# hitbc/panSVR

Measured on AMD Instinct MI355X. Metric: signal reads realigned/sec (150 bp PE); bit-exact CIGAR vs CPU ref, higher is better.
Workload: dtype u8/int32 (2-bit k-mers, 8-bit DP deltas, 32-bit scores); 1 GPU; configs[1]: 1000000 synthetic 150 bp PE signal read pairs per GPU vs 10000-anchor SV reference (11.8 Mbp), `panSVR aln` hot path; pairs_per_gpu=1000000, engines_per_gpu=1, in_process_rebases=0, index_hbm_bytes=2713674320, index_distribution=every rank uploads its own copy from host memory

## Files before the change

pansvr_amd/csrc/ksw_kernels.hip:

```cpp
#include <hip/hip_runtime.h>
#include <stdint.h>
#include "ksw_device.h"

namespace psvr {

__device__ __forceinline__ void write_ez(psvr_extz_t *o, const EzAcc &a, int n_cigar)
{
	o->max = a.max, o->zdropped = a.zdropped;
	o->max_q = a.max_q, o->max_t = a.max_t;
	o->mqe = a.mqe, o->mqe_t = a.mqe_t;
	o->mte = a.mte, o->mte_q = a.mte_q;
	o->score = a.score, o->n_cigar = n_cigar, o->reach_end = a.reach_end, o->reserved = 0;
}

__device__ __forceinline__ void wave_slot_take(int t, int tlen, const uint8_t *target, int neg_qe, int neg_qe2,
                                               int &u, int &v, int &x, int &y, int &x2, int &y2, int &s, int &H, int &tb)
{
	u = v = x = y = neg_qe, x2 = y2 = neg_qe2, s = 0, H = PSVR_KSW_NEG_INF;
	tb = t < tlen ? target[t] : 0;
}
template <int K, bool RING>
__device__ __forceinline__ void dp_wave_loop(const DpParams &P, const uint8_t *target, int lane, int qlen, int tlen, int w, int rowb, int n_rows,
                                             const uint8_t *QR, uint8_t *Pm, EzAcc &ez)
{
// ... 106 lines not shown
		last_st = st;
	}
}

template <int K>
__device__ __forceinline__ void dp_lean_loop(const DpParams &P, const uint8_t *target, int lane, int qlen, int tlen, int rowb, int n_rows,
                                             const uint8_t *QR, uint8_t *Pm, EzAcc &ez_out)
{
	const int neg_qe = s8(-P.q - P.e), neg_qe2 = s8(-P.q2 - P.e2);
	const int qe8 = s8(P.q + P.e), qe28 = s8(P.q2 + P.e2);
	const int with_cigar = !(P.flag & PSVR_EZ_SCORE_ONLY);
	int u[K], v[K], x[K], y[K], x2[K], y2[K], H[K], tb[K], mis[K];
#pragma unroll
	for (int c = 0; c < K; ++c) {
		const int t = c * 64 + lane;
		v[c] = x[c] = y[c] = neg_qe;
		x2[c] = y2[c] = neg_qe2;
		u[c] = dp_edge_gap(P, t);
		H[c] = -P.qe_pre;
		const int tc = t < tlen ? target[t] : 0;
		tb[c] = tc == P.m1 ? 0x100 : tc;
		mis[c] = tc == P.m1 ? P.sc_N : P.sc_mis;
	}
	__builtin_amdgcn_wave_barrier();
	int e_max = 0, e_max_t = -1, e_max_q = -1, e_mqe = PSVR_KSW_NEG_INF, e_mqe_t = -1, e_mte = PSVR_KSW_NEG_INF, e_mte_q = -1;
	int e_score = PSVR_KSW_NEG_INF, e_zd = 0, last_H = PSVR_KSW_NEG_INF;
	for (int r = 0; r < n_rows; ++r) {
		const int st0 = max(0, r - qlen + 1), en0 = min(tlen - 1, r);
		const int ur = dp_edge_gap(P, r);
		const int c_first = st0 >> 6, c_last = en0 >> 6;
		const int qbase = qlen - 1 - r;
		const unsigned prow = (unsigned)(r * rowb - (st0 & ~15));
		int h_prev = 0;
#pragma unroll
		for (int c = 0; c < K; ++c) {
			if (en0 > 0 && ((en0 - 1) >> 6) == c) h_prev = __builtin_amdgcn_readlane(H[c], (en0 - 1) & 63);
		}
		const int sel_t = en0 > 0 ? en0 : -1;
		int bh = (int)0x80000000;
		unsigned long long amask[K];
#pragma unroll
		for (int c = K - 1; c >= 0; --c) {
			amask[c] = 0;
			if (c < c_first || c > c_last) continue;
			const int t = c * 64 + lane;
			int cx = neg_qe, cv = ur, cx2 = neg_qe2;
			if (c > 0) {
				cx = __builtin_amdgcn_readlane(x[c - 1], 63);
				cv = __builtin_amdgcn_readlane(v[c - 1], 63);
				cx2 = __builtin_amdgcn_readlane(x2[c - 1], 63);
			}
			const int xt1 = dpp_wave_shr1(x[c], cx), vt1 = dpp_wave_shr1(v[c], cv), x2t1 = dpp_wave_shr1(x2[c], cx2);
			const int qb = QR[(unsigned)(qbase + t)];
			int sc = tb[c] == qb ? P.sc_mch : mis[c];
			sc = qb == P.m1 ? P.sc_N : sc;
			const int ut = u[c];
			int a = xt1 + vt1, b = y[c] + ut, a2 = x2t1 + vt1, b2 = y2[c] + ut;
			int z = max(max(sc, a), b);
			z = max(max(z, a2), b2);
			int d = 4;
			d = a2 == z ? 3 : d;
			d = b == z ? 2 : d;
			d = a == z ? 1 : d;
			d = sc == z ? 0 : d;
			z = min(z, P.sc_mch);
			const int un = z - vt1, vn = z - ut;
			const int zq = z - P.q, zq2 = z - P.q2;
			a -= zq, b -= zq, a2 -= zq2, b2 -= zq2;
			d |= (a > 0 ? 0x08 : 0) | (b > 0 ? 0x10 : 0) | (a2 > 0 ? 0x20 : 0) | (b2 > 0 ? 0x40 : 0);
			const int hn = t == sel_t ? h_prev + un : H[c] + vn;
			const bool act = (t >= st0) & (t <= en0);
			amask[c] = __ballot(act);
			if (act) {
				u[c] = un, v[c] = vn;
				x[c] = max(a, 0) - qe8, y[c] = max(b, 0) - qe8;
				x2[c] = max(a2, 0) - qe28, y2[c] = max(b2, 0) - qe28;
				H[c] = hn;
				if (with_cigar) Pm[prow + (unsigned)t] = (uint8_t)d;
				bh = max(bh, hn);
			}
		}
		const int max_H = wave_max_i32(bh);
		int n_top = 0, max_t = 0;
		unsigned long long top[K];
#pragma unroll
		for (int c = 0; c < K; ++c) {
			top[c] = 0;
			if (c < c_first || c > c_last) continue;
			top[c] = __ballot(H[c] == max_H) & amask[c];
			n_top += __popcll(top[c]);
			if (top[c]) max_t = c * 64 + __ffsll((unsigned long long)top[c]) - 1;
		}
		if (n_top != 1) {
			const int en1 = dp_diag_en1(st0, en0);
			unsigned bk = 0xffffffffu;
#pragma unroll
			for (int c = 0; c < K; ++c)
				if ((top[c] >> lane) & 1) bk = min(bk, dp_diag_rank<12>(c * 64 + lane, st0, en0, en1));
			max_t = dp_rank_col<12>(wave_min_u32(bk), st0, en0);
		}
		if (en0 == tlen - 1) {
			int H_en0 = 0;
#pragma unroll
			for (int c = 0; c < K; ++c)
				if ((en0 >> 6) == c) H_en0 = __builtin_amdgcn_readlane(H[c], en0 & 63);
			if (H_en0 > e_mte) e_mte = H_en0, e_mte_q = r - (((en0 + 16) & ~15) - 1);
			if (r == n_rows - 1) last_H = H_en0;
		}
		if (r - st0 == qlen - 1) {
			int H_st0 = 0;
#pragma unroll
			for (int c = 0; c < K; ++c)
				if ((st0 >> 6) == c) H_st0 = __builtin_amdgcn_readlane(H[c], st0 & 63);
			if (H_st0 > e_mqe) e_mqe = H_st0, e_mqe_t = st0;
		}
		if (max_H > e_max) {
			e_max = max_H, e_max_t = max_t, e_max_q = r - max_t;
		} else if (max_t >= e_max_t && r - max_t >= e_max_q) {
			const int tl = max_t - e_max_t, ql = (r - max_t) - e_max_q;
			const int l = tl > ql ? tl - ql : ql - tl;
			if (P.zdrop >= 0 && e_max - max_H > P.zdrop + l * P.e2) { e_zd = 1; break; }
		}
		if (r == n_rows - 1) e_score = last_H;
	}
	ez_out.max = e_max, ez_out.max_t = e_max_t, ez_out.max_q = e_max_q;
	ez_out.mqe = e_mqe, ez_out.mqe_t = e_mqe_t, ez_out.mte = e_mte, ez_out.mte_q = e_mte_q;
	ez_out.score = e_score, ez_out.zdropped = e_zd;
}

template <int K, bool PG, bool RING, int NW = kDpWaves>
__device__ __forceinline__ void extd2_wave_body(const DpBatch &B, const DpParams &P)
{
	extern __shared__ __align__(16) uint8_t lds_all[];
	const int wave = uni(threadIdx.x >> 6);
	const long long slot = (long long)blockIdx.x * NW + wave;
	if (slot >= B.n) return;
	uint8_t *lds = lds_all + (size_t)wave * B.lds_per_wave;
	const int pid = uni(B.idx[slot]);
	const int lane = threadIdx.x & 63;
	const int qlen = uni(B.qlen[pid]), tlen = uni(B.tlen[pid]);
	psvr_extz_t *out = B.ez + pid;
	EzAcc ez;
	ez.reset();
	if (P.skip || qlen <= 0 || tlen <= 0) {
		if (lane == 0) write_ez(out, ez, 0);
		return;
	}
	const uint8_t *query = B.qseq + uni64(B.q_off[pid]), *target = B.tseq + uni64(B.t_off[pid]);
	const int w = dp_band_w(qlen, tlen, P.w);
	const int rowb = uni(dp_n_col(qlen, tlen, P.w) * 16);
	const int n_rows = qlen + tlen - 1;
	const int qimg = (qlen + 16 + 15) & ~15;
	uint8_t *QR = lds;
	uint8_t *Pm = PG ? B.pslab + (uni64(B.p_off[pid]) << B.p_unit_shift) : lds + qimg;
	const int p_end = n_rows * rowb + 16;
	for (int i = lane; i < qimg; i += 64) QR[i] = i < qlen ? query[qlen - 1 - i] : 0;
	if (RING) {
		uint8_t *TG = lds + qimg;
		for (int i = lane; i < tlen; i += 64) TG[i] = target[i];
		dp_wave_loop<K, true>(P, TG, lane, qlen, tlen, w, rowb, n_rows, QR, Pm, ez);
	}
	else if (P.nowrap_ok && dp_band_never_binds(qlen, tlen, w)) dp_lean_loop<K>(P, target, lane, qlen, tlen, rowb, n_rows, QR, Pm, ez);
	else dp_wave_loop<K, false>(P, target, lane, qlen, tlen, w, rowb, n_rows, QR, Pm, ez);
	const int with_cigar = !(P.flag & PSVR_EZ_SCORE_ONLY);
	int n_cigar = 0;
	if (with_cigar) {
		if (PG) __threadfence_block();
		__builtin_amdgcn_wave_barrier();
		int i0, j0;
		if (trace_start(ez, P, qlen, tlen, i0, j0)) {
			uint32_t *stage_end = (uint32_t*)(Pm + p_end);
			n_cigar = traceback(i0, j0, qlen, tlen, w,
				[&](int r, int k) { return PG ? (int)__builtin_nontemporal_load(Pm + (size_t)r * rowb + k) : (int)Pm[r * rowb + k]; },
				[&](int k, uint32_t word) { if (lane == 0) stage_end[-1 - k] = word; });
			if (PG) __threadfence_block();
			__builtin_amdgcn_wave_barrier();
			uint32_t *dst = B.cigar + uni64(out->cigar_off);
			const bool rev = (P.flag & PSVR_EZ_REV_CIGAR) != 0;
			for (int m = lane; m < n_cigar; m += 64) {
				const uint32_t *src = rev ? stage_end - 1 - m : stage_end - n_cigar + m;
				dst[m] = PG ? __builtin_nontemporal_load(src) : *src;
			}
		}
	}
	if (lane == 0) write_ez(out, ez, n_cigar);
}
template <int K, bool PG>
__global__ __launch_bounds__(64 * kDpWaves) void extd2_reg_kernel(DpBatch B, DpParams P) { extd2_wave_body<K, PG, false>(B, P); }
template <int K>
__global__ __launch_bounds__(64 * kDpWaves) void extd2_ring_kernel(DpBatch B, DpParams P) { extd2_wave_body<K, true, true>(B, P); }
template __global__ void extd2_ring_kernel<3>(DpBatch, DpParams);
template __global__ void extd2_ring_kernel<4>(DpBatch, DpParams);
template <int K>
__global__ __launch_bounds__(64) void extd2_ring1_kernel(DpBatch B, DpParams P) { extd2_wave_body<K, true, true, 1>(B, P); }
template __global__ void extd2_ring1_kernel<3>(DpBatch, DpParams);
template __global__ void extd2_ring1_kernel<4>(DpBatch, DpParams);

template __global__ void extd2_reg_kernel<1, false>(DpBatch, DpParams);
template __global__ void extd2_reg_kernel<2, false>(DpBatch, DpParams);
template __global__ void extd2_reg_kernel<1, true>(DpBatch, DpParams);
template __global__ void extd2_reg_kernel<2, true>(DpBatch, DpParams);
template __global__ void extd2_reg_kernel<3, true>(DpBatch, DpParams);
template __global__ void extd2_reg_kernel<4, true>(DpBatch, DpParams);
template __global__ void extd2_reg_kernel<5, true>(DpBatch, DpParams);


__global__ __launch_bounds__(64) void extd2_tiny_kernel(DpBatch B, DpParams P, int max_rows)
{
	extern __shared__ __align__(16) uint32_t tiny_lds[];
	const int lane = threadIdx.x;
	const long long slot = (long long)blockIdx.x * 64 + lane;
	if (slot >= B.n) return;
	uint32_t *W0 = tiny_lds + lane, *W1 = tiny_lds + 16 * 64 + lane;
	uint8_t *PD = (uint8_t *)(tiny_lds + 2 * 16 * 64) + lane;
	const int pid = B.idx[slot];
	const int qlen = B.qlen[pid], tlen = B.tlen[pid];
	psvr_extz_t *out = B.ez + pid;
	EzAcc ez;
	ez.reset();
	if (P.skip || qlen <= 0 || tlen <= 0 || qlen > PSVR_DP_TINY_MAX || tlen > PSVR_DP_TINY_MAX || qlen + tlen - 1 > max_rows) { write_ez(out, ez, 0); return; }
	const uint8_t *query = B.qseq + B.q_off[pid], *target = B.tseq + B.t_off[pid];
	unsigned long long qp = 0, tp = 0;
	for (int i = 0; i < qlen; ++i) qp |= (unsigned long long)(query[i] & 15) << (4 * i);
	for (int i = 0; i < tlen; ++i) tp |= (unsigned long long)(target[i] & 15) << (4 * i);
	const int neg_qe = s8(-P.q - P.e), neg_qe2 = s8(-P.q2 - P.e2);
	const int qe8 = s8(P.q + P.e), qe28 = s8(P.q2 + P.e2);
	const int with_cigar = !(P.flag & PSVR_EZ_SCORE_ONLY);
	auto pack0 = [](int u, int v, int x, int y) { return (uint32_t)(u & 0xff) | (uint32_t)(v & 0xff) << 8 | (uint32_t)(x & 0xff) << 16 | (uint32_t)(y & 0xff) << 24; };
	auto pack1 = [](int x2, int y2, int h) { return (uint32_t)(x2 & 0xff) | (uint32_t)(y2 & 0xff) << 8 | (uint32_t)(h & 0xffff) << 16; };
	for (int t = 0; t < tlen; ++t) {
		W0[t * 64] = pack0(dp_edge_gap(P, t), neg_qe, neg_qe, neg_qe);
		W1[t * 64] = pack1(neg_qe2, neg_qe2, -P.qe_pre);
	}
	const int n_rows = qlen + tlen - 1;
	for (int r = 0; r < n_rows; ++r) {
		const int st0 = max(0, r - qlen + 1), en0 = min(tlen - 1, r);
		const int en1 = dp_diag_en1(st0, en0);
		int x1 = neg_qe, v1 = dp_edge_gap(P, r), x21 = neg_qe2, h1 = 0;
		if (st0 > 0) {
			const uint32_t a = W0[(st0 - 1) * 64], b = W1[(st0 - 1) * 64];
			v1 = s8(a >> 8), x1 = s8(a >> 16), x21 = s8(b), h1 = (int)(int16_t)(b >> 16);
		}
		int bh = (int)0x80000000, H_en0 = 0, H_st0 = 0;
		unsigned bk = 0xffffffffu;
		for (int t = st0; t <= en0; ++t) {
			const uint32_t a = W0[t * 64], b = W1[t * 64];
			const int ut = s8(a), vo = s8(a >> 8), xo = s8(a >> 16), yo = s8(a >> 24), x2o = s8(b), y2o = s8(b >> 8), ho = (int)(int16_t)(b >> 16);
			const int xt1 = x1, vt1 = v1, x2t1 = x21, hl = h1;
			x1 = xo, v1 = vo, x21 = x2o, h1 = ho;
			const int tc = (int)(tp >> (4 * t)) & 15, qc = (int)(qp >> (4 * (r - t))) & 15;
			int sc = tc == qc ? P.sc_mch : P.sc_mis;
			sc = (tc == P.m1 || qc == P.m1) ? P.sc_N : sc;
			int za = xt1 + vt1, zb = yo + ut, za2 = x2t1 + vt1, zb2 = y2o + ut;
			int z = max(max(sc, za), zb);
			z = max(max(z, za2), zb2);
			int d = 4;
			d = za2 == z ? 3 : d;
			d = zb == z ? 2 : d;
			d = za == z ? 1 : d;
			d = sc == z ? 0 : d;
			z = min(z, P.sc_mch);
			const int un = z - vt1, vn = z - ut;
			const int zq = z - P.q, zq2 = z - P.q2;
			za -= zq, zb -= zq, za2 -= zq2, zb2 -= zq2;
			d |= (za > 0 ? 0x08 : 0) | (zb > 0 ? 0x10 : 0) | (za2 > 0 ? 0x20 : 0) | (zb2 > 0 ? 0x40 : 0);
			const int hn = (t == en0 && en0 > 0) ? hl + un : ho + vn;
			W0[t * 64] = pack0(un, vn, max(za, 0) - qe8, max(zb, 0) - qe8);
			W1[t * 64] = pack1(max(za2, 0) - qe28, max(zb2, 0) - qe28, hn);
			if (with_cigar) PD[(r * 16 + t) * 64] = (uint8_t)d;
			if (t == en0) H_en0 = hn;
			if (t == st0) H_st0 = hn;
			const unsigned rank = dp_diag_rank<12>(t, st0, en0, en1);
			if (hn > bh || (hn == bh && rank < bk)) bh = hn, bk = rank;
		}
		const int max_t = dp_rank_col<12>(bk, st0, en0);
		if (ez.end_diagonal(r, qlen, tlen, st0, en0, H_st0, H_en0, bh, max_t, P.zdrop, P.e2)) break;
	}
	int n_cigar = 0;
	if (with_cigar) {
		int i0, j0;
		if (trace_start(ez, P, qlen, tlen, i0, j0)) {
			const int w = dp_band_w(qlen, tlen, P.w);
			n_cigar = traceback(i0, j0, qlen, tlen, w,
				[&](int r, int k) { return (int)PD[(r * 16 + k) * 64]; },
				[&](int k, uint32_t word) { (k < 16 ? W0[k * 64] : W1[(k - 16) * 64]) = word; });
			uint32_t *dst = B.cigar + out->cigar_off;
			const bool rev = (P.flag & PSVR_EZ_REV_CIGAR) != 0;
			for (int m = 0; m < n_cigar; ++m) {
				const int k = rev ? m : n_cigar - 1 - m;
				dst[m] = k < 16 ? W0[k * 64] : W1[(k - 16) * 64];
			}
		}
	}
	write_ez(out, ez, n_cigar);
}

static constexpr int kTeamWaves = 3;
template <int LANES, int CPL, int LEAN>
__global__ __launch_bounds__(64) __attribute__((amdgpu_waves_per_eu(kTeamWaves, 8))) void extd2_team_kernel(DpBatch B, DpParams P, TeamPlan T)
{
	static_assert(CPL == 4 || CPL == 8 || CPL == 16, "columns per lane: direction bytes go out as dwords");
	constexpr int SW = CPL * LANES, PB = 64 / LANES;
	constexpr int kNone = (int)0x80000000;
	const int lane = threadIdx.x, team = lane / LANES, ql = lane % LANES;
	__shared__ int sc_lut[64];
	{
		const int tcode = lane >> 3, qcode = lane & 7;
		sc_lut[lane] = 8 * ((tcode == P.m1 || qcode == P.m1) ? P.sc_N : (tcode == qcode ? P.sc_mch : P.sc_mis)) + 4;
	}
	__builtin_amdgcn_wave_barrier();
	int cls = 0;
	while (cls + 1 < T.n_classes && (int)blockIdx.x >= T.first_block[cls + 1]) ++cls;
	const int n_strips16 = T.n_strips16[cls];
	const long long slot = (long long)((int)blockIdx.x - T.first_block[cls]) * PB + team;
	const bool live = slot < T.count[cls];
	int pid = 0, qlen = 0, tlen = 0;
	if (live) pid = B.idx[T.first_slot[cls] + slot], qlen = B.qlen[pid], tlen = B.tlen[pid];
	const int n_strips = (n_strips16 * 16 + SW - 1) / SW;
	const int qmax = wave_max_i32(qlen > 0 ? qlen : 0);
	const int ksteps = uni(qmax + LANES - 1);
	const int k_last = uni(-wave_max_i32(live && qlen > 0 ? -qlen : (int)0x80000000)) - 1;
	const int R = ksteps, NR = qmax + SW * n_strips + 1;
	const unsigned long long need = dp_team_ws_bytes(qmax, n_strips16, LANES, CPL);
	const unsigned long long base = T.ws_base[cls] + (unsigned long long)((int)blockIdx.x - T.first_block[cls]) * T.ws_need[cls];
	const bool bad_shape = qlen <= 0 || tlen <= 0 || (tlen + SW - 1) / SW > n_strips;
	if (!live) return;
	if (base + need > B.ws_cap && B.err) *B.err = 20;
	if (P.skip || bad_shape || base + need > B.ws_cap) return;
	uint8_t *w0 = B.ws + base;
	const size_t offE = (size_t)(64 * CPL) * n_strips * R;
	uint8_t *const uE0 = w0 + offE, *const uE1 = w0 + offE + (size_t)4 * PB * NR;
	uint8_t *const uD = w0 + offE + (size_t)8 * PB * NR, *const uD23 = uD + (size_t)4 * PB * NR;
	const unsigned lc = (unsigned)CPL * (unsigned)lane, t4 = 4u * (unsigned)team;
	auto at4 = [=](uint8_t *ub, int r) -> int & { return *(int *)(ub + (size_t)r * (4 * PB) + t4); };
	auto atD2 = [=](int r) -> short & { return *(short *)(uD23 + (size_t)r * (4 * PB) + t4); };
	auto atD3 = [=](int r) -> short & { return *(short *)(uD23 + (size_t)r * (4 * PB) + t4 + 2); };
	const uint8_t *query = B.qseq + B.q_off[pid], *target = B.tseq + B.t_off[pid];
	const int with_cigar = !(P.flag & PSVR_EZ_SCORE_ONLY);
	const int neg_qe = s8(-P.q - P.e), neg_qe2 = s8(-P.q2 - P.e2);
	const int x_init = 8 * neg_qe + 3, y_init = 8 * neg_qe + 2, x2_init = 8 * neg_qe2 + 1, y2_init = 8 * neg_qe2;
	const int z_cap = 8 * P.sc_mch + 7;
	const int q_m8 = 8 * P.q - 8, q2_m8 = 8 * P.q2 - 8;
	const int cx = 8 - 8 * s8(P.q + P.e), cx2 = 8 - 8 * s8(P.q2 + P.e2);
	const int long_thres = P.long_thres, ur_short = s8(-P.e), ur_at = s8(P.long_diff), ur_long = s8(-P.e2);
	auto ur_of = [=](int r) { return r == 0 ? neg_qe : r < long_thres ? ur_short : r == long_thres ? ur_at : ur_long; };
	auto h_above = [&](int t) {
		int h = -P.qe_pre;
		const int lt = P.long_thres;
		if (t >= 1) {
			if (lt >= 1) h += t < lt ? t * s8(-P.e) : (lt - 1) * s8(-P.e) + s8(P.long_diff) + (t - lt) * s8(-P.e2);
			else h += t * s8(-P.e2);
		}
		return h;
	};
	auto frank = [](int p) { return (((p << 12) + p) & 0x3fff) ^ 0x3fff; };
	const int ns = (tlen + SW - 1) / SW;
	for (int sv = 0; sv < ns; ++sv) {
		const int s = uni(sv);
		const int c0 = SW * s;
		const int ncols = tlen - c0 < SW ? tlen - c0 : SW;
		const int jb = CPL * ql, cb = c0 + jb;
		const int jx = tlen - 1 - cb;
		const bool own = (unsigned)jx < (unsigned)CPL;
		int U[CPL], V[CPL], X[CPL], Y[CPL], X2[CPL], Y2[CPL], H[CPL], TC[CPL];
		int M[CPL], K[CPL], G[CPL];
		bool inr[CPL];
#pragma unroll
		for (int jj = 0; jj < CPL; ++jj) {
			U[jj] = 8 * ur_of(cb + jj);
			V[jj] = 8 * neg_qe, X[jj] = x_init, Y[jj] = y_init, X2[jj] = x2_init, Y2[jj] = y2_init;
			H[jj] = 8 * h_above(cb + jj);
			inr[jj] = jb + jj < ncols;
			TC[jj] = inr[jj] ? (target[cb + jj] & 7) * 32 : 0;
			M[jj] = kNone, G[jj] = frank(cb + jj);
			const int d = cb + jj - ql;
			const int st = max(0, d - qlen + 1), en = min(tlen - 1, d);
			K[jj] = st + ((en - st) & ~3) - cb;
		}
		(void)M, (void)K, (void)G;
		uint8_t *const Ein = (s & 1) ? uE0 : uE1, *const Eout = (s & 1) ? uE1 : uE0;
		unsigned e_prev = 0;
		unsigned dirw[CPL / 4];
		int d_cur = kNone, out_prev = kNone;
		if (s > 0) {
			e_prev = (unsigned)at4(Ein, 0);
			if (!LEAN && 0 <= ksteps - LANES) d_cur = at4(uD, c0);
		}
		unsigned q_cur = ql == 0 ? query[0] : 0u;
		for (int kv = 0; kv < LANES - 1; ++kv) {
			const int k = uni(kv);
#define TEAM_MASKED 1
#define TEAM_TOPROW 1
#include "ksw_row_step.inc"
#undef TEAM_MASKED
#undef TEAM_TOPROW
		}
		{
			const int k = LANES - 1;
#define TEAM_MASKED 0
#define TEAM_TOPROW 1
#include "ksw_row_step.inc"
#undef TEAM_MASKED
#undef TEAM_TOPROW
		}
		for (int kv = LANES; kv < ksteps; ++kv) {
			const int k = uni(kv);
#define TEAM_MASKED 0
#define TEAM_TOPROW 0
#include "ksw_row_step.inc"
#undef TEAM_MASKED
#undef TEAM_TOPROW
		}
		if (with_cigar) {
			uint32_t *const dst = (uint32_t *)(w0 + (size_t)(s * R + ksteps - 1) * (64 * CPL) + lc);
#pragma unroll
			for (int g = 0; g < CPL / 4; ++g) dst[g] = dirw[g];
		}
		if (LEAN) { __threadfence_block(); continue; }
		if (LANES > 1) {
			const int inc = __builtin_amdgcn_update_dpp(kNone, out_prev, 0x101, 0xf, 0xf, false);
			const int m0 = __builtin_amdgcn_update_dpp(kNone, M[0], 0x101, 0xf, 0xf, false);
			M[CPL - 2] = max(M[CPL - 2], ql == LANES - 1 ? kNone : inc);
			M[CPL - 1] = max(M[CPL - 1], ql == LANES - 1 ? kNone : m0);
		}
#pragma unroll
		for (int jj = 0; jj < CPL; ++jj)
			if (jj > 0 || ql == 0) at4(uD, ksteps - ql + cb + jj) = M[jj];
		__threadfence_block();
	}
}

static constexpr int kFinishWaves = 8;
template <int LANES, int CPL, int LEAN>
__global__ __launch_bounds__(64) __attribute__((amdgpu_waves_per_eu(1, kFinishWaves))) void extd2_team_finish_kernel(DpBatch B, DpParams P, TeamPlan T)
{
	constexpr int SW = CPL * LANES, PB = 64 / LANES, kWinRows = 8;
	__shared__ uint32_t win[kWinRows * (CPL / 4) * 64];
	const int lane = threadIdx.x, team = lane % PB;
	const int tb = (int)((blockIdx.x * 64u + (unsigned)lane) / (unsigned)PB);
	const bool in_grid = tb < T.first_block[T.n_classes];
	int cls = 0;
	while (cls + 1 < T.n_classes && tb >= T.first_block[cls + 1]) ++cls;
	const int n_strips16 = T.n_strips16[cls];
	const long long slot = (long long)(tb - T.first_block[cls]) * PB + team;
	const bool live = in_grid && slot < T.count[cls];
	int pid = 0, qlen = 0, tlen = 0;
	if (live) pid = B.idx[T.first_slot[cls] + slot], qlen = B.qlen[pid], tlen = B.tlen[pid];
	const int n_strips = (n_strips16 * 16 + SW - 1) / SW;
	int qmax = qlen > 0 ? qlen : 0;
#pragma unroll
	for (int d = 1; d < PB; d <<= 1) qmax = max(qmax, __shfl_xor(qmax, d, 64));
	const int ksteps = qmax + LANES - 1;
	const int R = ksteps, NR = qmax + SW * n_strips + 1;
	const unsigned long long need = dp_team_ws_bytes(qmax, n_strips16, LANES, CPL);
	const unsigned long long base = T.ws_base[cls] + (unsigned long long)(tb - T.first_block[cls]) * T.ws_need[cls];
	if (!live) return;
	psvr_extz_t *out = B.ez + pid;
	EzAcc ez;
	ez.reset();
	const bool bad_shape = qlen <= 0 || tlen <= 0 || (tlen + SW - 1) / SW > n_strips;
	if (P.skip || bad_shape || base + need > B.ws_cap) { write_ez(out, ez, 0); return; }
	uint8_t *w0 = B.ws + base;
	const size_t offE = (size_t)(64 * CPL) * n_strips * R;
	uint8_t *const uD = w0 + offE + (size_t)8 * PB * NR, *const uD23 = uD + (size_t)4 * PB * NR;
	const unsigned t4 = 4u * (unsigned)team;
	auto at4 = [=](uint8_t *ub, int r) -> int & { return *(int *)(ub + (size_t)r * (4 * PB) + t4); };
	const int with_cigar = !(P.flag & PSVR_EZ_SCORE_ONLY);
	const int n_rows = qlen + tlen - 1;
	bool stop = false;
	for (int r0 = 0; r0 < n_rows && !stop; r0 += 8) {
		int kd[8], h2[8], h3[8];
#pragma unroll
		for (int u = 0; u < 8; ++u) {
			const int r = min(r0 + u, n_rows - 1);
			const int w23 = at4(uD23, r);
			kd[u] = LEAN ? 0 : at4(uD, r), h2[u] = (int)(short)(w23 & 0xffff), h3[u] = w23 >> 16;
		}
#pragma unroll
		for (int u = 0; u < 8; ++u) {
			const int r = r0 + u;
			if (r >= n_rows || stop) continue;
			const int st0 = max(0, r - qlen + 1), en0 = min(tlen - 1, r);
			const int key = kd[u];
			const int max_H = key >> 16;
			const int H_en0 = h2[u];
			const int max_t = H_en0 == max_H ? en0 : st0 + ((0x7fff - (key & 0xffff)) & 4095);
			if (en0 == tlen - 1 && H_en0 > ez.mte) ez.mte = H_en0, ez.mte_q = r - (((en0 + 16) & ~15) - 1);
			if (r - st0 == qlen - 1 && h3[u] > ez.mqe) ez.mqe = h3[u], ez.mqe_t = st0;
			if (!LEAN && ez.apply_zdrop(max_H, r, max_t, P.zdrop, P.e2)) stop = true;
			else if (r == n_rows - 1) ez.score = H_en0;
		}
	}
	int n_cigar = 0;
	if (with_cigar) {
		int i0, j0;
		if (trace_start(ez, P, qlen, tlen, i0, j0)) {
			const int w = dp_band_w(qlen, tlen, P.w);
			const uint8_t *pb = w0 + team * SW;
			uint32_t *stage = (uint32_t *)(w0 + offE) + team;
			int win_row = -1, win_grp = -1;
			n_cigar = traceback(i0, j0, qlen, tlen, w,
				[&](int r, int k) {
					const int t = k + (max(0, r - qlen + 1) & ~15), row = r - t, grp = t / CPL;
					if (grp != win_grp || row > win_row || row <= win_row - kWinRows) {
						const int s = grp / LANES, gl = grp % LANES;
						const uint8_t *src = pb + (size_t)(s * R + row + gl) * (64 * CPL) + gl * CPL;
						uint32_t tmp[kWinRows][CPL / 4];
#pragma unroll
						for (int d = 0; d < kWinRows; ++d)
#pragma unroll
							for (int u = 0; u < CPL / 4; ++u) tmp[d][u] = d <= row ? ((const uint32_t *)(src - (size_t)d * (64 * CPL)))[u] : 0u;
#pragma unroll
						for (int d = 0; d < kWinRows; ++d)
#pragma unroll
							for (int u = 0; u < CPL / 4; ++u) win[(d * (CPL / 4) + u) * 64 + lane] = tmp[d][u];
						win_row = row, win_grp = grp;
					}
					const int x = t % CPL;
					const unsigned b = (win[((win_row - row) * (CPL / 4) + (x >> 2)) * 64 + lane] >> (8 * (x & 3))) & 0xffu, n = ~b;
					return (int)((4u - ((b >> 4) & 7u)) | ((n >> 3) & 1u) << 3 | ((n >> 2) & 1u) << 4 | ((n >> 1) & 1u) << 5 | (n & 1u) << 6);
				},
				[&](int k, uint32_t word) { stage[(size_t)k * PB] = word; });
			uint32_t *dst = B.cigar + out->cigar_off;
			const bool rev = (P.flag & PSVR_EZ_REV_CIGAR) != 0;
			for (int m = 0; m < n_cigar; ++m) dst[m] = stage[(size_t)(rev ? m : n_cigar - 1 - m) * PB];
		}
	}
	write_ez(out, ez, n_cigar);
}
template __global__ void extd2_team_kernel<kDpTeamLanes, kDpTeamCpl, 0>(DpBatch, DpParams, TeamPlan);
template __global__ void extd2_team_finish_kernel<kDpTeamLanes, kDpTeamCpl, 0>(DpBatch, DpParams, TeamPlan);
template __global__ void extd2_team_kernel<kDpTeamLanes, kDpTeamCpl, 1>(DpBatch, DpParams, TeamPlan);
template __global__ void extd2_team_finish_kernel<kDpTeamLanes, kDpTeamCpl, 1>(DpBatch, DpParams, TeamPlan);

struct GenK {
	int neg_qe, neg_qe2, qe8, qe28;
	int qe;
	uint8_t qe2b, max_scb, qb8;
	int with_cigar, approx_max, right;
};
__device__ __forceinline__ GenK gen_consts(const DpParams &P)
{
	GenK k;
	k.neg_qe = s8(-P.q - P.e), k.neg_qe2 = s8(-P.q2 - P.e2), k.qe8 = s8(P.q + P.e), k.qe28 = s8(P.q2 + P.e2);
	k.qe = P.q + P.e;
	k.qe2b = (uint8_t)((P.q + P.e) * 2), k.max_scb = (uint8_t)(P.mat[0] + (P.q + P.e) * 2), k.qb8 = (uint8_t)P.q;
	k.with_cigar = !(P.flag & PSVR_EZ_SCORE_ONLY), k.approx_max = !!(P.flag & PSVR_EZ_APPROX_MAX);
	k.right = k.with_cigar && (P.flag & PSVR_EZ_RIGHT);
	return k;
}

template <int VAR, class IDX>
struct GenImage {
	static constexpr int NARR = VAR == 0 ? 7 : 5;
	uint8_t *base;
	IDX T, img;
	int8_t *u8, *v8, *x8, *y8, *x28, *y28, *sa;
	uint8_t *sf, *qr;
	int32_t *H;
	__device__ __forceinline__ void place(uint8_t *at, int qlen, int tlen)
	{
		base = at;
		T = ((IDX)tlen + 15) / 16 * 16;
		const IDX QL = ((IDX)qlen + 15) / 16 * 16;
		u8 = (int8_t*)at, v8 = u8 + T, x8 = v8 + T, y8 = x8 + T;
		x28 = VAR == 0 ? y8 + T : nullptr, y28 = VAR == 0 ? x28 + T : nullptr;
		sa = VAR == 0 ? y28 + T : y8 + T;
		sf = (uint8_t*)(sa + T), qr = sf + T;
		img = NARR * T + T + QL + 16;
		H = (int32_t*)(at + ((img + 15) & ~(IDX)15));
	}
	__device__ __forceinline__ void init(int tid, int nthreads, const uint8_t *query, const uint8_t *target, int qlen, int tlen, const GenK &k) const
	{
		for (IDX i = tid; i < img; i += nthreads) {
			const IDX a = i / T;
			uint8_t val = 0;
			if (VAR == 0) { if (a < 4) val = (uint8_t)k.neg_qe; else if (a < 6) val = (uint8_t)k.neg_qe2; }
			if (a == NARR) { const IDX t = i - NARR * T; val = t < tlen ? target[t] : 0; }
			if (a > NARR)  { const IDX j = i - (NARR + 1) * T; val = j < qlen ? query[qlen - 1 - j] : 0; }
			base[i] = val;
		}
		for (IDX i = tid; i < T; i += nthreads) H[i] = PSVR_KSW_NEG_INF;
	}
	__device__ __forceinline__ int du(const GenK &k, int t) const { return VAR == 0 ? (int)u8[t] : (int)(uint8_t)u8[t] - k.qe; }
	__device__ __forceinline__ int dv(const GenK &k, int t) const { return VAR == 0 ? (int)v8[t] : (int)(uint8_t)v8[t] - k.qe; }
	__device__ __forceinline__ int h_first(const GenK &k, const DpParams &P) const { return dv(k, 0) - (VAR == 0 ? P.qe_pre : k.qe); }
};

template <int VAR, class IMG>
__device__ __forceinline__ void gen_left_boundary(const IMG &I, const GenK &k, const DpParams &P, int r, int st, int last_st, int last_en, int &x1, int &x21, int &v1)
{
	x21 = 0;
	if (VAR == 0) {
		if (st > 0) {
			if (st - 1 >= last_st && st - 1 <= last_en) x1 = I.x8[st - 1], x21 = I.x28[st - 1], v1 = I.v8[st - 1];
			else x1 = k.neg_qe, x21 = k.neg_qe2, v1 = k.neg_qe;
		} else x1 = k.neg_qe, x21 = k.neg_qe2, v1 = dp_edge_gap(P, r);
	} else {
		if (st > 0) {
			if (st - 1 >= last_st && st - 1 <= last_en) x1 = I.x8[st - 1], v1 = I.v8[st - 1];
			else x1 = v1 = 0;
		} else x1 = 0, v1 = r ? s8(P.q) : 0;
	}
}

template <int VAR, class IMG>
__device__ __forceinline__ void gen_row_override(const IMG &I, const GenK &k, const DpParams &P, int r)
{
	if (VAR == 0) I.y8[r] = k.neg_qe, I.y28[r] = k.neg_qe2, I.u8[r] = dp_edge_gap(P, r);
	else I.y8[r] = 0, I.u8[r] = r ? (int8_t)k.qb8 : 0;
}

struct GenLate { int t, sc; };
template <bool DEFER, class IMG>
__device__ __forceinline__ GenLate gen_scores(const IMG &I, const DpParams &P, int qlen, int r, int st0, int en0, int tid, int nthreads)
{
	const uint8_t *qrr = I.qr + (qlen - 1 - r);
	GenLate late = {-1, 0};
	if (!(P.flag & PSVR_EZ_GENERIC_SC)) {
		const int fresh_end = dp_fresh_end(st0, en0);
		for (int t = st0 + tid; t <= fresh_end; t += nthreads) {
			const uint8_t sq = I.sf[t], sq2 = qrr[t];
			int sc = sq == sq2 ? P.sc_mch : P.sc_mis;
			if (sq == (uint8_t)P.m1 || sq2 == (uint8_t)P.m1) sc = P.sc_N;
			if (!DEFER || t < I.T) I.sa[t] = (int8_t)sc;
			else late.t = t, late.sc = sc;
		}
	} else {
		for (int t = st0 + tid; t <= en0; t += nthreads) I.sa[t] = P.mat[I.sf[t] * P.m + qrr[t]];
	}
	return late;
}

struct GenCell { int u, v, x, y, x2, y2, d; };
template <int VAR, class IMG>
__device__ __forceinline__ GenCell gen_cell(const IMG &I, const GenK &k, const DpParams &P, int t, int st, int x1, int x21, int v1)
{
	GenCell c = {0, 0, 0, 0, 0, 0, 0};
	int d = 0;
	if (VAR == 0) {
		int xt1 = t == st ? x1 : (int)I.x8[t - 1], vt1 = t == st ? v1 : (int)I.v8[t - 1], x2t1 = t == st ? x21 : (int)I.x28[t - 1];
		int z = I.sa[t], ut = I.u8[t];
		int a = s8(xt1 + vt1), b = s8(I.y8[t] + ut), a2 = s8(x2t1 + vt1), b2 = s8(I.y28[t] + ut);
		if (!k.right) {
			if (a > z)  d = 1, z = a;
			if (b > z)  d = 2, z = b;
			if (a2 > z) d = 3, z = a2;
			if (b2 > z) d = 4, z = b2;
		} else {
			d = z > a ? 0 : 1;  z = z > a ? z : a;
			d = z > b ? d : 2;  z = z > b ? z : b;
			d = z > a2 ? d : 3; z = z > a2 ? z : a2;
			d = z > b2 ? d : 4; z = z > b2 ? z : b2;
		}
		z = min(z, P.sc_mch);
		c.u = z - vt1, c.v = z - ut;
		int tmp = s8(z - P.q);
		a = s8(a - tmp), b = s8(b - tmp);
		tmp = s8(z - P.q2);
		a2 = s8(a2 - tmp), b2 = s8(b2 - tmp);
		c.x = max(a, 0) - k.qe8, c.y = max(b, 0) - k.qe8, c.x2 = max(a2, 0) - k.qe28, c.y2 = max(b2, 0) - k.qe28;
		if (!k.right) d |= (a > 0 ? 0x08 : 0) | (b > 0 ? 0x10 : 0) | (a2 > 0 ? 0x20 : 0) | (b2 > 0 ? 0x40 : 0);
		else d |= (a >= 0 ? 0x08 : 0) | (b >= 0 ? 0x10 : 0) | (a2 >= 0 ? 0x20 : 0) | (b2 >= 0 ? 0x40 : 0);
	} else {
		const int j = t - st;
		unsigned x1w = (unsigned)x1, v1w = (unsigned)v1;
		uint8_t xt1 = j == 0 ? 0 : (uint8_t)I.x8[t - 1], vt1 = j == 0 ? 0 : (uint8_t)I.v8[t - 1];
		if (j < 4) xt1 |= (uint8_t)(x1w >> (8 * j)), vt1 |= (uint8_t)(v1w >> (8 * j));
		uint8_t z = (uint8_t)((uint8_t)I.sa[t] + k.qe2b), a = (uint8_t)(xt1 + vt1), ut = (uint8_t)I.u8[t], b = (uint8_t)((uint8_t)I.y8[t] + ut);
		if (!k.with_cigar) {
			z = (int8_t)z > 0 ? z : 0; z = z > a ? z : a;
		} else if (!k.right) {
			d = (int8_t)a > (int8_t)z ? 1 : 0;
			z = (int8_t)z > 0 ? z : 0; z = z > a ? z : a;
			if ((int8_t)b > (int8_t)z) d = 2;
		} else {
			d = (int8_t)z > (int8_t)a ? 0 : 1;
			z = (int8_t)z > 0 ? z : 0; z = z > a ? z : a;
			if (!((int8_t)z > (int8_t)b)) d = 2;
		}
		z = z > b ? z : b;
		z = z < k.max_scb ? z : k.max_scb;
		c.u = (uint8_t)(z - vt1), c.v = (uint8_t)(z - ut);
		z = (uint8_t)(z - k.qb8);
		a = (uint8_t)(a - z), b = (uint8_t)(b - z);
		if (!k.right) {
			c.x = (int8_t)a > 0 ? (int8_t)a : 0; d |= (int8_t)a > 0 ? 0x08 : 0;
			c.y = (int8_t)b > 0 ? (int8_t)b : 0; d |= (int8_t)b > 0 ? 0x10 : 0;
		} else {
			c.x = (int8_t)a < 0 ? 0 : (int8_t)a; d |= (int8_t)a < 0 ? 0 : 0x08;
			c.y = (int8_t)b < 0 ? 0 : (int8_t)b; d |= (int8_t)b < 0 ? 0 : 0x10;
		}
	}
	c.d = d;
	return c;
}
template <int VAR, class IMG>
__device__ __forceinline__ void gen_store_cell(const IMG &I, int t, const GenCell &c)
{
	I.u8[t] = (int8_t)c.u, I.v8[t] = (int8_t)c.v, I.x8[t] = (int8_t)c.x, I.y8[t] = (int8_t)c.y;
	if (VAR == 0) I.x28[t] = (int8_t)c.x2, I.y28[t] = (int8_t)c.y2;
}

template <class IMG>
__device__ __forceinline__ int gen_h_en0(const IMG &I, const GenK &k, int en0)
{
	const int uen = I.du(k, en0), ven = I.dv(k, en0);
	return en0 > 0 ? I.H[en0 - 1] + uen : I.H[en0] + ven;
}
template <int RS, class IMG>
__device__ __forceinline__ void gen_exact_h_partial(const IMG &I, const GenK &k, int st0, int en0, int h_en0, int tid, int nthreads, int &bh, unsigned &bk)
{
	const int en1 = dp_diag_en1(st0, en0);
	bh = (int)0x80000000, bk = 0xffffffffu;
	for (int t = st0 + tid; t <= en0; t += nthreads) {
		const int h = t == en0 ? h_en0 : I.H[t] + I.dv(k, t);
		I.H[t] = h;
		const unsigned rank = dp_diag_rank<RS>(t, st0, en0, en1);
		if (h > bh || (h == bh && rank < bk)) bh = h, bk = rank;
// ... 231 lines not shown
```

pansvr_amd/csrc/ksw_row_step.inc:

```
		const int i = k - ql;
		if (with_cigar && k > 0) {
			uint32_t *const dst = (uint32_t *)(w0 + (size_t)(s * R + k - 1) * (64 * CPL) + lc);
#pragma unroll
			for (int g = 0; g < CPL / 4; ++g) dst[g] = dirw[g];
		}
		const bool act = (unsigned)i < (unsigned)qlen;
		const unsigned q_nxt = (unsigned)(i + 1) < (unsigned)qlen ? query[i + 1] : 0u;
		const int qc4 = (int)((q_cur << 2) & 0x1cu);
		int vl = 0, xl = 0, x2l = 0;
		if (LANES > 1) {
			vl = __builtin_amdgcn_update_dpp(0, V[CPL - 1], 0x111, 0xf, 0xf, false), xl = __builtin_amdgcn_update_dpp(0, X[CPL - 1], 0x111, 0xf, 0xf, false);
			x2l = __builtin_amdgcn_update_dpp(0, X2[CPL - 1], 0x111, 0xf, 0xf, false);
			if (!LEAN) {
				const int inc = __builtin_amdgcn_update_dpp(kNone, out_prev, 0x101, 0xf, 0xf, false);
				M[CPL - 2] = max(M[CPL - 2], ql == LANES - 1 ? kNone : inc);
			}
		}
		unsigned e_next = 0;
		int d_nxt = kNone;
		if (s > 0) {
			e_next = (unsigned)at4(Ein, k + 1);
			if (!LEAN && k + 1 <= ksteps - LANES) d_nxt = at4(uD, c0 + k + 1);
		}
		if (ql == 0) {
			if (s > 0) vl = __builtin_amdgcn_sbfe((int)e_prev, 0, 8) << 3, xl = (__builtin_amdgcn_sbfe((int)e_prev, 8, 8) << 3) | 3, x2l = (__builtin_amdgcn_sbfe((int)e_prev, 16, 8) << 3) | 1;
			else vl = 8 * ur_of(i), xl = x_init, x2l = x2_init;
		}
		const int rowc = qlen - 1 - i, rc = rowc - cb, g_row = frank(rowc);
		int acc[CPL];
#pragma unroll
		for (int jj = 0; jj < CPL; ++jj) {
			const int xt1 = jj ? X[jj ? jj - 1 : 0] : xl, vt1 = jj ? V[jj ? jj - 1 : 0] : vl, x2t1 = jj ? X2[jj ? jj - 1 : 0] : x2l;
			const int sc = *(const int *)((const char *)sc_lut + (TC[jj] | qc4));
			const int ut = U[jj];
			int za = xt1 + vt1, zb = Y[jj] + ut, za2 = x2t1 + vt1, zb2 = Y2[jj] + ut;
			int m = max(max(sc, za), zb);
			m = max(max(m, za2), zb2);
			const int z = min(m, z_cap) & ~7;
			const int un = z - vt1, vn = z - ut;
			const int zq = z - q_m8, zq2 = z - q2_m8;
			za -= zq, zb -= zq, za2 -= zq2, zb2 -= zq2;
			int a = m;
			a = (int)__builtin_amdgcn_alignbit((unsigned)a, (unsigned)za, 31);
			a = (int)__builtin_amdgcn_alignbit((unsigned)a, (unsigned)zb, 31);
			a = (int)__builtin_amdgcn_alignbit((unsigned)a, (unsigned)za2, 31);
			a = (int)__builtin_amdgcn_alignbit((unsigned)a, (unsigned)zb2, 31);
			acc[jj] = a;
			const int hn = H[jj] + vn;
			int key = 0;
			if (!LEAN) {
				const int low = ((jj - K[jj]) & 0x4000) | (jj <= rc ? G[jj] : g_row);
				key = (int)((unsigned)hn << 13) | low;
			}
			if (!TEAM_MASKED || act) {
				U[jj] = un, V[jj] = vn;
				X[jj] = max(za, -5) + cx, Y[jj] = max(zb, -6) + cx;
				X2[jj] = max(za2, -7) + cx2, Y2[jj] = max(zb2, -8) + cx2;
				H[jj] = hn;
			}
			if (!LEAN) M[jj] = max(M[jj], (act & inr[jj]) ? key : kNone);
		}
		const int out = LEAN ? 0 : M[0];
		if (!LEAN && ql == 0) at4(uD, c0 + k) = max(out, d_cur);
		if (!LEAN) {
			const int d_in = i + cb + CPL;
			const int st_in = max(0, d_in - qlen + 1), en_in = min(tlen - 1, d_in);
#pragma unroll
			for (int jj = 0; jj + 1 < CPL; ++jj) M[jj] = M[jj + 1], K[jj] = K[jj + 1] + 0;
			M[CPL - 1] = kNone, K[CPL - 1] = st_in + ((en_in - st_in) & ~3) - cb;
		}
#pragma unroll
		for (int g = 0; g < CPL; g += 4) {
			const unsigned lo = __builtin_amdgcn_perm((unsigned)acc[g + 1], (unsigned)acc[g], 0x0c0c0400u);
			const unsigned hi = __builtin_amdgcn_perm((unsigned)acc[g + 3], (unsigned)acc[g + 2], 0x04000c0cu);
			dirw[g >> 2] = lo | hi;
		}
		if (ql == LANES - 1 && s + 1 < ns && act)
			at4(Eout, i) = (int)((((unsigned)V[CPL - 1] >> 3) & 0xffu) | ((((unsigned)X[CPL - 1] >> 3) & 0xffu) << 8) | ((((unsigned)X2[CPL - 1] >> 3) & 0xffu) << 16));
		if (TEAM_TOPROW && i == 0) {
#pragma unroll
			for (int jj = 0; jj < CPL; ++jj) if (inr[jj]) atD2(cb + jj) = (short)(H[jj] >> 3);
		}
		if (own & act) {
			int hx = H[CPL - 1];
#pragma unroll
			for (int u = CPL - 2; u >= 0; --u) hx = jx == u ? H[u] : hx;
			atD2(i + tlen - 1) = (short)(hx >> 3);
		}
		if (k >= k_last && i == qlen - 1) {
#pragma unroll
			for (int jj = 0; jj < CPL; ++jj) if (inr[jj]) atD3(qlen - 1 + cb + jj) = (short)(H[jj] >> 3);
		}
		out_prev = out, e_prev = e_next, d_cur = d_nxt, q_cur = q_nxt;
```

Measured before the change: 374.3 million reads/s.

## Software-pipeline row-step loads and defer boundary stores via carried register

Restructures the team DP row step so the next row's query, E-carry and D loads are issued unconditionally with clamped indices inside a sched_barrier-fenced block, away from the compute. In LEAN mode the right-edge E and D2 boundary values are kept in a carry register and written one step later with precomputed offsets, which removes the dependent stores from the critical path. Prologue loads of target bytes, query, E and D are hoisted ahead of the register initialisation. This hides LDS and global latency between rows. The cost is extra unconditional loads, more live registers, and a heavier dependence on compiler scheduling barriers.

```diff
diff --git a/pansvr_amd/csrc/ksw_kernels.hip b/pansvr_amd/csrc/ksw_kernels.hip
--- a/pansvr_amd/csrc/ksw_kernels.hip
+++ b/pansvr_amd/csrc/ksw_kernels.hip
@@ -432,6 +432,7 @@
 	static_assert(CPL == 4 || CPL == 8 || CPL == 16, "columns per lane: direction bytes go out as dwords");
 	constexpr int SW = CPL * LANES, PB = 64 / LANES;
 	constexpr int kNone = (int)0x80000000;
+	constexpr bool CARRY = LEAN != 0;
 	const int lane = threadIdx.x, team = lane / LANES, ql = lane % LANES;
 	__shared__ int sc_lut[64];
 	{
@@ -492,6 +493,18 @@
 		const int jb = CPL * ql, cb = c0 + jb;
 		const int jx = tlen - 1 - cb;
 		const bool own = (unsigned)jx < (unsigned)CPL;
+		const bool eown = ql == LANES - 1 && s + 1 < ns;
+		const unsigned qlen_e = eown ? (unsigned)qlen : 0u, qlen_o = own ? (unsigned)qlen : 0u;
+		const int eoff = (int)t4 - ql * (4 * PB), ooff = (int)t4 + (tlen - 1 - ql) * (4 * PB);
+		uint8_t *const Ein = (s & 1) ? uE0 : uE1, *const Eout = (s & 1) ? uE1 : uE0;
+		unsigned tb[CPL];
+#pragma unroll
+		for (int jj = 0; jj < CPL; ++jj) tb[jj] = target[min(cb + jj, tlen - 1)];
+		unsigned q_cur = query[0];
+		unsigned e_prev = (unsigned)at4(Ein, 0);
+		int d_cur = kNone, out_prev = kNone;
+		if (!LEAN) d_cur = at4(uD, c0);
+		__builtin_amdgcn_sched_barrier(0);
 		int U[CPL], V[CPL], X[CPL], Y[CPL], X2[CPL], Y2[CPL], H[CPL], TC[CPL];
 		int M[CPL], K[CPL], G[CPL];
 		bool inr[CPL];
@@ -501,22 +514,17 @@
 			V[jj] = 8 * neg_qe, X[jj] = x_init, Y[jj] = y_init, X2[jj] = x2_init, Y2[jj] = y2_init;
 			H[jj] = 8 * h_above(cb + jj);
 			inr[jj] = jb + jj < ncols;
-			TC[jj] = inr[jj] ? (target[cb + jj] & 7) * 32 : 0;
 			M[jj] = kNone, G[jj] = frank(cb + jj);
 			const int d = cb + jj - ql;
 			const int st = max(0, d - qlen + 1), en = min(tlen - 1, d);
 			K[jj] = st + ((en - st) & ~3) - cb;
 		}
 		(void)M, (void)K, (void)G;
-		uint8_t *const Ein = (s & 1) ? uE0 : uE1, *const Eout = (s & 1) ? uE1 : uE0;
-		unsigned e_prev = 0;
+		__builtin_amdgcn_sched_barrier(0);
+#pragma unroll
+		for (int jj = 0; jj < CPL; ++jj) TC[jj] = inr[jj] ? (int)(tb[jj] & 7) * 32 : 0;
 		unsigned dirw[CPL / 4];
-		int d_cur = kNone, out_prev = kNone;
-		if (s > 0) {
-			e_prev = (unsigned)at4(Ein, 0);
-			if (!LEAN && 0 <= ksteps - LANES) d_cur = at4(uD, c0);
-		}
-		unsigned q_cur = ql == 0 ? query[0] : 0u;
+		unsigned carry = 0;
 		for (int kv = 0; kv < LANES - 1; ++kv) {
 			const int k = uni(kv);
 #define TEAM_MASKED 1
@@ -545,6 +553,11 @@
 			uint32_t *const dst = (uint32_t *)(w0 + (size_t)(s * R + ksteps - 1) * (64 * CPL) + lc);
 #pragma unroll
 			for (int g = 0; g < CPL / 4; ++g) dst[g] = dirw[g];
+		}
+		if (CARRY) {
+			const int ip = ksteps - 1 - ql;
+			if ((unsigned)ip < qlen_e) at4(Eout, ip) = (int)carry;
+			if ((unsigned)ip < qlen_o) atD2(ip + tlen - 1) = (short)carry;
 		}
 		if (LEAN) { __threadfence_block(); continue; }
 		if (LANES > 1) {
diff --git a/pansvr_amd/csrc/ksw_row_step.inc b/pansvr_amd/csrc/ksw_row_step.inc
--- a/pansvr_amd/csrc/ksw_row_step.inc
+++ b/pansvr_amd/csrc/ksw_row_step.inc
@@ -1,11 +1,7 @@
 		const int i = k - ql;
-		if (with_cigar && k > 0) {
-			uint32_t *const dst = (uint32_t *)(w0 + (size_t)(s * R + k - 1) * (64 * CPL) + lc);
-#pragma unroll
-			for (int g = 0; g < CPL / 4; ++g) dst[g] = dirw[g];
-		}
 		const bool act = (unsigned)i < (unsigned)qlen;
-		const unsigned q_nxt = (unsigned)(i + 1) < (unsigned)qlen ? query[i + 1] : 0u;
+		asm volatile("" : "+v"(q_cur), "+v"(e_prev));
+		if (!LEAN) asm volatile("" : "+v"(d_cur));
 		const int qc4 = (int)((q_cur << 2) & 0x1cu);
 		int vl = 0, xl = 0, x2l = 0;
 		if (LANES > 1) {
@@ -16,16 +12,26 @@
 				M[CPL - 2] = max(M[CPL - 2], ql == LANES - 1 ? kNone : inc);
 			}
 		}
-		unsigned e_next = 0;
-		int d_nxt = kNone;
-		if (s > 0) {
-			e_next = (unsigned)at4(Ein, k + 1);
-			if (!LEAN && k + 1 <= ksteps - LANES) d_nxt = at4(uD, c0 + k + 1);
-		}
+		const int d_row = (!LEAN && s > 0 && k <= ksteps - LANES) ? d_cur : kNone;
 		if (ql == 0) {
 			if (s > 0) vl = __builtin_amdgcn_sbfe((int)e_prev, 0, 8) << 3, xl = (__builtin_amdgcn_sbfe((int)e_prev, 8, 8) << 3) | 3, x2l = (__builtin_amdgcn_sbfe((int)e_prev, 16, 8) << 3) | 1;
 			else vl = 8 * ur_of(i), xl = x_init, x2l = x2_init;
 		}
+		__builtin_amdgcn_sched_barrier(0);
+		if (with_cigar && (!TEAM_MASKED || k > 0)) {
+			uint32_t *const dst = (uint32_t *)(w0 + (size_t)(s * R + k - 1) * (64 * CPL) + lc);
+#pragma unroll
+			for (int g = 0; g < CPL / 4; ++g) dst[g] = dirw[g];
+		}
+		if (CARRY) {
+			const long long rowb = (long long)(k - 1) * (4 * PB);
+			if ((unsigned)(i - 1) < qlen_e) *(int *)(Eout + rowb + eoff) = (int)carry;
+			if ((unsigned)(i - 1) < qlen_o) *(short *)(uD23 + rowb + ooff) = (short)carry;
+		}
+		q_cur = query[min(TEAM_MASKED ? max(i + 1, 0) : i + 1, qlen - 1)];
+		e_prev = (unsigned)at4(Ein, k + 1);
+		if (!LEAN) d_cur = at4(uD, c0 + k + 1);
+		__builtin_amdgcn_sched_barrier(0);
 		const int rowc = qlen - 1 - i, rc = rowc - cb, g_row = frank(rowc);
 		int acc[CPL];
 #pragma unroll
@@ -61,7 +67,7 @@
 			if (!LEAN) M[jj] = max(M[jj], (act & inr[jj]) ? key : kNone);
 		}
 		const int out = LEAN ? 0 : M[0];
-		if (!LEAN && ql == 0) at4(uD, c0 + k) = max(out, d_cur);
+		if (!LEAN && ql == 0) at4(uD, c0 + k) = max(out, d_row);
 		if (!LEAN) {
 			const int d_in = i + cb + CPL;
 			const int st_in = max(0, d_in - qlen + 1), en_in = min(tlen - 1, d_in);
@@ -75,20 +81,32 @@
 			const unsigned hi = __builtin_amdgcn_perm((unsigned)acc[g + 3], (unsigned)acc[g + 2], 0x04000c0cu);
 			dirw[g >> 2] = lo | hi;
 		}
-		if (ql == LANES - 1 && s + 1 < ns && act)
-			at4(Eout, i) = (int)((((unsigned)V[CPL - 1] >> 3) & 0xffu) | ((((unsigned)X[CPL - 1] >> 3) & 0xffu) << 8) | ((((unsigned)X2[CPL - 1] >> 3) & 0xffu) << 16));
+		if (CARRY) {
+			unsigned c = 0;
+			if (eown) c = (((unsigned)V[CPL - 1] >> 3) & 0xffu) | ((((unsigned)X[CPL - 1] >> 3) & 0xffu) << 8) | ((((unsigned)X2[CPL - 1] >> 3) & 0xffu) << 16);
+			if (own) {
+				int hx = H[CPL - 1];
+#pragma unroll
+				for (int u = CPL - 2; u >= 0; --u) hx = jx == u ? H[u] : hx;
+				c = (unsigned)(hx >> 3);
+			}
+			carry = c;
+		} else {
+			if (eown & act)
+				at4(Eout, i) = (int)((((unsigned)V[CPL - 1] >> 3) & 0xffu) | ((((unsigned)X[CPL - 1] >> 3) & 0xffu) << 8) | ((((unsigned)X2[CPL - 1] >> 3) & 0xffu) << 16));
+			if (own & act) {
+				int hx = H[CPL - 1];
+#pragma unroll
+				for (int u = CPL - 2; u >= 0; --u) hx = jx == u ? H[u] : hx;
+				atD2(i + tlen - 1) = (short)(hx >> 3);
+			}
+		}
 		if (TEAM_TOPROW && i == 0) {
 #pragma unroll
 			for (int jj = 0; jj < CPL; ++jj) if (inr[jj]) atD2(cb + jj) = (short)(H[jj] >> 3);
-		}
-		if (own & act) {
-			int hx = H[CPL - 1];
-#pragma unroll
-			for (int u = CPL - 2; u >= 0; --u) hx = jx == u ? H[u] : hx;
-			atD2(i + tlen - 1) = (short)(hx >> 3);
 		}
 		if (k >= k_last && i == qlen - 1) {
 #pragma unroll
 			for (int jj = 0; jj < CPL; ++jj) if (inr[jj]) atD3(qlen - 1 + cb + jj) = (short)(H[jj] >> 3);
 		}
-		out_prev = out, e_prev = e_next, d_cur = d_nxt, q_cur = q_nxt;
+		out_prev = out;
```

After: 379.4 million reads/s, median of 6. 1.4% higher.
